# ibm-granite/dolomite-engine

Measured on AMD Instinct MI355X. Metric: tokens/sec/node GPTDolomite-3B bf16 seq4096 padding-free, higher is better.
Workload: dtype bf16; 1 GPU; gptdolomite-3b-bf16-seq4096-paddingfree-pretrain; model=GPTDolomite-3B, global_batch=16, seq_len=4096, parallelism=dp1

## Files before the change

### dolomite_engine_amd/csrc/attention.hip

```cpp

#include "common.h"

typedef __bf16 bf16x8 __attribute__((ext_vector_type(8)));
typedef float f32x4 __attribute__((ext_vector_type(4)));
typedef uint32_t u32x4 __attribute__((ext_vector_type(4)));

#define MFMA16(a, b, c) __builtin_amdgcn_mfma_f32_16x16x32_bf16((a), (b), (c), 0, 0, 0)

#define DOL_LOG2E 1.44269504088896340736f
#define DOL_LN2 0.69314718055994530942f

#define PI23(q) (((q) & ~12) | ((((q) >> 2) & 1) << 3) | ((((q) >> 3) & 1) << 2))

typedef __bf16 bf16x4 __attribute__((ext_vector_type(4)));


__device__ __forceinline__ bf16x8 lds_tr16_bfrag(const __bf16* img, int rowbase, int S, int d0, int lane) {
    const int g8 = (lane >> 4) * 8;
    const int jj = (lane >> 2) & 3;
    const int cc = (lane & 3) * 4;
    unsigned a0 = (unsigned)(size_t)(img + PI23(rowbase + g8 + jj) * S + d0 + cc);
    unsigned a1 = (unsigned)(size_t)(img + PI23(rowbase + g8 + 4 + jj) * S + d0 + cc);
    bf16x4 lo, hi;
    asm volatile(
// ... 381 lines not shown
    return dol_last_error();
}

static int fa_varlen_fwd_dispatch(dolomite_stream_t stream,
                                  const void* q, const void* k, const void* v,
                                  void* o, float* lse,
                                  const int32_t* seq_begin, const int32_t* seq_end,
                                  int batch, int max_seqlen, int64_t T,
                                  int H, int Hkv, int D, int G,
                                  int64_t q_tstride, int64_t q_gstride,
                                  int64_t k_tstride, int64_t k_hstride,
                                  int64_t v_tstride, int64_t v_hstride,
                                  float scale, int dtype, float p_drop, uint64_t seed) {
    if (dtype != DOLOMITE_BF16) return 9010;
    if (D > 128) return 9011;
    if (!(scale > 0.f)) return 9015;
    int max_tiles = (max_seqlen + 127) / 128;
    hipStream_t s = (hipStream_t)stream;
#define CASE(DP, DROP)                                                                               \
    return launch_fa_fwd<DP, DROP>(s, (const __bf16*)q, (const __bf16*)k, (const __bf16*)v,          \
                                   (__bf16*)o, lse, seq_begin, seq_end, batch, T, H, Hkv, D, G, q_tstride, \
                                   q_gstride, k_tstride, k_hstride, v_tstride, v_hstride, max_tiles, \
                                   scale, p_drop, seed)
    if (p_drop > 0.f) {
        if (D <= 32) CASE(32, true);
        if (D <= 64) CASE(64, true);
        if (D <= 96) CASE(96, true);
        CASE(128, true);
    }
    if (D <= 32) CASE(32, false);
    if (D <= 64) CASE(64, false);
    if (D <= 96) CASE(96, false);
    CASE(128, false);
#undef CASE
}

extern "C" int dolomite_fa_varlen_fwd(dolomite_stream_t stream,
                                      const void* q, const void* k, const void* v,
                                      void* o, float* lse,
                                      const int32_t* cu_seqlens, int batch, int max_seqlen, int64_t T,
                                      int H, int Hkv, int D, int G,
                                      int64_t q_tstride, int64_t q_gstride,
                                      int64_t k_tstride, int64_t k_hstride,
                                      int64_t v_tstride, int64_t v_hstride,
                                      float scale, int dtype) {
    return fa_varlen_fwd_dispatch(stream, q, k, v, o, lse, cu_seqlens, cu_seqlens + 1, batch, max_seqlen, T,
                                  H, Hkv, D, G, q_tstride, q_gstride, k_tstride, k_hstride,
                                  v_tstride, v_hstride, scale, dtype, 0.f, 0);
}

extern "C" int dolomite_fa_varlen_fwd_dropout(dolomite_stream_t stream,
                                              const void* q, const void* k, const void* v,
                                              void* o, float* lse,
                                              const int32_t* cu_seqlens, int batch, int max_seqlen, int64_t T,
                                              int H, int Hkv, int D, int G,
                                              int64_t q_tstride, int64_t q_gstride,
                                              int64_t k_tstride, int64_t k_hstride,
                                              int64_t v_tstride, int64_t v_hstride,
                                              float scale, int dtype, float p_drop, uint64_t seed) {
    if (!drop_p_valid(p_drop)) return 9013;
    return fa_varlen_fwd_dispatch(stream, q, k, v, o, lse, cu_seqlens, cu_seqlens + 1, batch, max_seqlen, T,
                                  H, Hkv, D, G, q_tstride, q_gstride, k_tstride, k_hstride,
                                  v_tstride, v_hstride, scale, dtype, p_drop, seed);
}


template <typename T>
__global__ void __launch_bounds__(256) fa_bwd_preprocess_kernel(
    const T* __restrict__ o, const T* __restrict__ dout, float* __restrict__ delta,
    int64_t T_total, int H, int D, int64_t o_ts, int64_t do_ts) {
    int64_t row = ((int64_t)blockIdx.x * 4) + (threadIdx.x >> 6);
    int lane = threadIdx.x & 63;
    if (row >= T_total * H) return;
    int64_t t = row / H;
    int h = (int)(row % H);
    const T* op = o + t * o_ts + (int64_t)h * D;
    const T* dp = dout + t * do_ts + (int64_t)h * D;
    float acc = 0.f;
    for (int d = lane * 2; d + 1 < D; d += 128) {
        float o0[2], d0[2];
        VecIO<T, 2>::load(op + d, o0);
        VecIO<T, 2>::load(dp + d, d0);
        acc += o0[0] * d0[0] + o0[1] * d0[1];
    }
    if (D & 1) {
        int d = D - 1;
        if (lane == 0) acc += load_as_f32(op + d) * load_as_f32(dp + d);
    }
    acc = wave_reduce_sum(acc);
    if (lane == 0) delta[(int64_t)h * T_total + t] = acc;
}

__global__ void __launch_bounds__(256) fa_bwd_preprocess_tiled(
    const __bf16* __restrict__ o, const __bf16* __restrict__ dout, float* __restrict__ delta,
    int64_t T_total, int H, int D, int TOK) {
    extern __shared__ float part[];
    const int64_t hd = (int64_t)H * D;
    const int64_t base = (int64_t)blockIdx.x * TOK * hd;
    const int64_t total = T_total * hd;
    const int np = (int)(TOK * hd / 8);
#pragma unroll 4
    for (int p = threadIdx.x; p < np; p += 256) {
        int64_t flat = base + (int64_t)p * 8;
        float acc = 0.f;
        if (flat + 8 <= total) {
            bf16x8 ov = *(const bf16x8*)(o + flat);
            bf16x8 dv = *(const bf16x8*)(dout + flat);
#pragma unroll
            for (int e = 0; e < 8; ++e) acc += (float)ov[e] * (float)dv[e];
        }
        part[p] = acc;
    }
    __syncthreads();
    const int slots = TOK * H;
    const int dp8 = D / 8;
    for (int s = threadIdx.x; s < slots; s += 256) {
        float a = 0.f;
        const float* ps = &part[s * dp8];
        for (int i = 0; i < dp8; ++i) a += ps[i];
        int tl = s / H, h = s - tl * H;
        int64_t t = (int64_t)blockIdx.x * TOK + tl;
        if (t < T_total) delta[(int64_t)h * T_total + t] = a;
    }
}

extern "C" int dolomite_fa_bwd_preprocess(dolomite_stream_t stream,
                                          const void* o, const void* dout, float* delta,
                                          int64_t T, int H, int D,
                                          int64_t o_tstride, int64_t do_tstride, int dtype) {
    const int64_t hd = (int64_t)H * D;
    int TOK = 16;
    while (TOK > 1 && TOK * hd * 4 / 8 > 65536) TOK /= 2;
    if (dtype == DOLOMITE_BF16 && D % 8 == 0 && o_tstride == hd && do_tstride == hd && T > 0 &&
        TOK * hd * 4 / 8 <= 65536) {
        dim3 grid((uint32_t)((T + TOK - 1) / TOK)), block(256);
        size_t shmem = (size_t)(TOK * hd / 8) * sizeof(float);
        hipLaunchKernelGGL((fa_bwd_preprocess_tiled), grid, block, shmem, (hipStream_t)stream,
                           (const __bf16*)o, (const __bf16*)dout, delta, T, H, D, TOK);
        return dol_last_error();
    }
    int64_t rows = T * H;
    dim3 grid((uint32_t)((rows + 3) / 4)), block(256);
    if (dtype == DOLOMITE_BF16)
        hipLaunchKernelGGL((fa_bwd_preprocess_kernel<uint16_t>), grid, block, 0, (hipStream_t)stream,
                           (const uint16_t*)o, (const uint16_t*)dout, delta, T, H, D, o_tstride, do_tstride);
    else
        hipLaunchKernelGGL((fa_bwd_preprocess_kernel<float>), grid, block, 0, (hipStream_t)stream,
                           (const float*)o, (const float*)dout, delta, T, H, D, o_tstride, do_tstride);
    return dol_last_error();
}



template <int DPAD, bool DROPOUT>
__global__ void __launch_bounds__(512, DPAD <= 96 ? 4 : 2) fa_bwd_dkv_kernel(
    const __bf16* __restrict__ q, const __bf16* __restrict__ k, const __bf16* __restrict__ v,
    const __bf16* __restrict__ dout, const float* __restrict__ lse, const float* __restrict__ delta,
    float* __restrict__ dk_acc, float* __restrict__ dv_acc,
    const int32_t* __restrict__ seq_begin, const int32_t* __restrict__ seq_end,
    int H, int Hkv, int D, int G,
    int64_t q_ts, int64_t q_gs, int64_t k_ts, int64_t k_hs, int64_t v_ts, int64_t v_hs,
    int64_t do_ts, int64_t T_total, float scale,
    uint32_t seed_lo, uint32_t seed_hi, uint32_t drop_thr, float drop_rp) {
    constexpr int KCH = DPAD / 32;
    constexpr int DCH = DPAD / 16;

    int tile_id = blockIdx.x, b = blockIdx.y, h = blockIdx.z;
    xcd_remap_tile_bh(tile_id, b, h);
    const int kvh = h / G;
    const int s0 = __builtin_amdgcn_readfirstlane(seq_begin[b]);
    const int L = __builtin_amdgcn_readfirstlane(seq_end[b]) - s0;
    const int ks = tile_id * 128;
    if (ks >= L) return;

    const int lane = threadIdx.x & 63;
    const int wave = threadIdx.x >> 6;
    const int lr = lane & 15;
    const int lg = lane >> 4;

    constexpr int SQ = DPAD + 16;
    constexpr int STS = 128 + 4;
    extern __shared__ char smem_raw[];
    __bf16* Qlds = (__bf16*)smem_raw;
    __bf16* dOl = Qlds + 64 * SQ;
    __bf16* dSTl = dOl + 64 * SQ;
    __bf16* PTl = dSTl + 64 * STS;

    const int kend = min(L, ks + 128);

    const int krow = ks + wave * 16 + lr;
    const bool kvalid = krow < kend;
    bf16x8 kfr[KCH], vfr[KCH];
#pragma unroll
    for (int kc = 0; kc < KCH; ++kc) {
        int d0 = kc * 32 + lg * 8;
        const __bf16* kp = k + (int64_t)(s0 + (kvalid ? krow : 0)) * k_ts + (int64_t)kvh * k_hs + d0;
        kfr[kc] = load_bf16x8_guard(kp, d0, D, kvalid);
        const __bf16* vp = v + (int64_t)(s0 + (kvalid ? krow : 0)) * v_ts + (int64_t)kvh * v_hs + d0;
        vfr[kc] = load_bf16x8_guard(vp, d0, D, kvalid);
    }

    f32x4 dvr[DCH], dkr[DCH];
#pragma unroll
    for (int dc = 0; dc < DCH; ++dc) {
        dvr[dc] = {0.f, 0.f, 0.f, 0.f};
        dkr[dc] = {0.f, 0.f, 0.f, 0.f};
    }

    uint32_t drop_cw[4];
    if constexpr (DROPOUT) {
        const uint32_t drop_hw = drop_head_word(seed_hi, (uint32_t)h);
#pragma unroll
        for (int r = 0; r < 4; ++r)
            drop_cw[r] = drop_col_word(drop_hw, (uint32_t)(s0 + ks + wave * 16 + lg * 4 + r));
    }

    const int tr_jj = (lane >> 2) & 3;
    const int tr_g8 = (lane >> 4) * 8;
    const int tr_cc = (lane & 3) * 4;
    const unsigned aQ0 = (unsigned)(size_t)(Qlds + PI23(tr_g8 + tr_jj) * SQ + tr_cc);
    const unsigned aQ1 = (unsigned)(size_t)(Qlds + PI23(tr_g8 + 4 + tr_jj) * SQ + tr_cc);
    const unsigned aDS0 = (unsigned)(size_t)(dSTl + PI23(tr_g8 + tr_jj) * STS + wave * 16 + tr_cc);
    const unsigned aDS1 = (unsigned)(size_t)(dSTl + PI23(tr_g8 + 4 + tr_jj) * STS + wave * 16 + tr_cc);
    constexpr int DO_IMM = 64 * SQ * 2;
    constexpr int PT_IMM = 64 * STS * 2;
    static_assert(DO_IMM + 32 * SQ * 2 + 16 * 2 < 65536, "ds offset range");
    static_assert(PT_IMM + 32 * STS * 2 + 16 * 2 < 65536, "ds offset range");

    if (__builtin_amdgcn_readfirstlane(threadIdx.x) >= 256) __builtin_amdgcn_s_setprio(1);

    const int qt0 = ks / 64;
    const int nqt = (L + 63) / 64;
    const int64_t q_hoff = (int64_t)(h / G) * q_gs + (int64_t)(h % G) * D;
    const int64_t do_hoff = (int64_t)h * D;

    if (D < DPAD) {
        for (int pidx = threadIdx.x; pidx < 64 * (DPAD - D) / 8; pidx += 512) {
            int qq = pidx / ((DPAD - D) / 8);
            int d0 = D + (pidx % ((DPAD - D) / 8)) * 8;
            bf16x8 z = {};
            *(bf16x8*)&Qlds[PI23(qq) * SQ + d0] = z;
            *(bf16x8*)&dOl[PI23(qq) * SQ + d0] = z;
        }
    }

    const unsigned st_magic = (1u << 22) / (unsigned)(D / 8) + 1;
    for (int qt = qt0; qt < nqt; ++qt) {
        const int qs = qt * 64;
        __syncthreads();
        {
            const int pieces = 64 * DPAD / 8;
            if (qs + 64 <= L) {
                for (int pidx = threadIdx.x; pidx < 64 * D / 8; pidx += 512) {
                    int qq = (int)(((unsigned)pidx * st_magic) >> 22);
                    int d0 = (pidx - qq * (D / 8)) * 8;
                    *(bf16x8*)&Qlds[PI23(qq) * SQ + d0] =
                        *(const bf16x8*)(q + (int64_t)(s0 + qs + qq) * q_ts + q_hoff + d0);
                    *(bf16x8*)&dOl[PI23(qq) * SQ + d0] =
                        *(const bf16x8*)(dout + (int64_t)(s0 + qs + qq) * do_ts + do_hoff + d0);
                }
            } else {
                for (int pidx = threadIdx.x; pidx < pieces; pidx += 512) {
                    int qq = pidx / (DPAD / 8);
                    int d0 = (pidx % (DPAD / 8)) * 8;
                    bool valid = (qs + qq) < L;
                    const __bf16* qp = q + (int64_t)(s0 + (valid ? qs + qq : 0)) * q_ts + q_hoff + d0;
                    *(bf16x8*)&Qlds[PI23(qq) * SQ + d0] = load_bf16x8_guard(qp, d0, D, valid);
                    const __bf16* dp = dout + (int64_t)(s0 + (valid ? qs + qq : 0)) * do_ts + do_hoff + d0;
                    *(bf16x8*)&dOl[PI23(qq) * SQ + d0] = load_bf16x8_guard(dp, d0, D, valid);
                }
            }
        }
        __syncthreads();

        const bool full_tile = (ks + wave * 16 + 16 <= qs + 1) && (kend == ks + 64) && (qs + 64 <= L);
#pragma unroll
        for (int cb = 0; cb < 4; ++cb) {
            f32x4 st = {0.f, 0.f, 0.f, 0.f};
            f32x4 dpt = {0.f, 0.f, 0.f, 0.f};
#pragma unroll
            for (int kc = 0; kc < KCH; ++kc) {
                int d0 = kc * 32 + lg * 8;
                bf16x8 qb = *(const bf16x8*)&Qlds[(cb * 16 + PI23(lr)) * SQ + d0];
                st = MFMA16(kfr[kc], qb, st);
                bf16x8 db = *(const bf16x8*)&dOl[(cb * 16 + PI23(lr)) * SQ + d0];
                dpt = MFMA16(vfr[kc], db, dpt);
            }
            const int qpos = qs + cb * 16 + lr;
            const bool qok = qpos < L;
            float lsev = qok ? lse[(int64_t)h * T_total + s0 + qpos] * DOL_LOG2E : 0.f;
            float delv = qok ? delta[(int64_t)h * T_total + s0 + qpos] : 0.f;
            bf16x4 pvv, dsv;
            uint32_t drop_rw = 0;
            if constexpr (DROPOUT) drop_rw = drop_row_word(seed_lo, (uint32_t)(s0 + qpos));
            if (__builtin_amdgcn_readfirstlane(full_tile ? 1 : 0)) {
#pragma unroll
                for (int r = 0; r < 4; ++r) {
                    float pv = exp2f(st[r] * (scale * DOL_LOG2E) - lsev);
                    if constexpr (DROPOUT) {
                        const bool keep = drop_keep_words(drop_rw, drop_cw[r], drop_thr);
                        pvv[r] = (__bf16)(keep ? pv : 0.f);
                        dsv[r] = (__bf16)(pv * ((keep ? dpt[r] * drop_rp : 0.f) - delv) * scale);
                    } else {
                        pvv[r] = (__bf16)pv;
                        dsv[r] = (__bf16)(pv * (dpt[r] - delv) * scale);
                    }
                }
            } else {
#pragma unroll
                for (int r = 0; r < 4; ++r) {
                    const int kpos = ks + wave * 16 + lg * 4 + r;
                    bool ok = qok && kpos < kend && kpos <= qpos;
                    float pv = ok ? exp2f(st[r] * (scale * DOL_LOG2E) - lsev) : 0.f;
                    if constexpr (DROPOUT) {
                        const bool keep = drop_keep_words(drop_rw, drop_cw[r], drop_thr);
                        float ds = ok ? pv * ((keep ? dpt[r] * drop_rp : 0.f) - delv) * scale : 0.f;
                        pvv[r] = (__bf16)(keep ? pv : 0.f);
                        dsv[r] = (__bf16)ds;
                    } else {
                        float ds = ok ? pv * (dpt[r] - delv) * scale : 0.f;
                        pvv[r] = (__bf16)pv;
                        dsv[r] = (__bf16)ds;
                    }
                }
            }
            const int srow = PI23(cb * 16 + lr) * STS + wave * 16 + lg * 4;
            *(bf16x4*)&PTl[srow] = pvv;
            *(bf16x4*)&dSTl[srow] = dsv;
        }

        {
            asm volatile("s_waitcnt lgkmcnt(0)" ::: "memory");
            __builtin_amdgcn_sched_barrier(0);
            bf16x4 a_lo[2], a_hi[2];
            tr16_issue<PT_IMM>(aDS0, aDS1, a_lo[0], a_hi[0]);
            tr16_issue<PT_IMM + 32 * STS * 2>(aDS0, aDS1, a_lo[1], a_hi[1]);
            bf16x4 blo[3], bhi[3];
            tr16_issue<DO_IMM>(aQ0, aQ1, blo[0], bhi[0]);
            tr16_issue<DO_IMM + ((1 / DCH) * 32 * SQ + (1 % DCH) * 16) * 2>(aQ0, aQ1, blo[1], bhi[1]);
            lgkm_wait4<4>(a_lo[0], a_hi[0], a_lo[1], a_hi[1]);
            bf16x8 af0 = tr16_join8(a_lo[0], a_hi[0]);
            bf16x8 af1 = tr16_join8(a_lo[1], a_hi[1]);
#define DKV_HALF(i, IMM, ACC, AF0, AF1)                                                                 \
    if constexpr ((i) < 2 * DCH) {                                                                      \
        constexpr int kc2_ = (i) / DCH, dc_ = (i) % DCH;                                                \
        if constexpr ((i) + 2 < 2 * DCH) {                                                              \
            constexpr int kn_ = ((i) + 2) / DCH, dn_ = ((i) + 2) % DCH;                                 \
            tr16_issue<(kn_ * 32 * SQ + dn_ * 16) * 2 + (IMM)>(aQ0, aQ1, blo[((i) + 2) % 3], bhi[((i) + 2) % 3]); \
            lgkm_wait2<4>(blo[(i) % 3], bhi[(i) % 3]);                                                  \
        } else if constexpr ((i) + 1 < 2 * DCH) {                                                       \
            lgkm_wait2<2>(blo[(i) % 3], bhi[(i) % 3]);                                                  \
        } else {                                                                                        \
            lgkm_wait2<0>(blo[(i) % 3], bhi[(i) % 3]);                                                  \
        }                                                                                               \
        ACC[dc_] = MFMA16(kc2_ ? (AF1) : (AF0), tr16_join8(blo[(i) % 3], bhi[(i) % 3]), ACC[dc_]);      \
    }
#define DKV_A(i) DKV_HALF(i, DO_IMM, dvr, af0, af1)
            DKV_A(0) DKV_A(1) DKV_A(2) DKV_A(3)
            DKV_A(4) DKV_A(5) DKV_A(6) DKV_A(7)
            DKV_A(8) DKV_A(9) DKV_A(10) DKV_A(11)
            DKV_A(12) DKV_A(13) DKV_A(14) DKV_A(15)
#undef DKV_A
            tr16_issue<0>(aDS0, aDS1, a_lo[0], a_hi[0]);
            tr16_issue<32 * STS * 2>(aDS0, aDS1, a_lo[1], a_hi[1]);
            tr16_issue<0>(aQ0, aQ1, blo[0], bhi[0]);
            tr16_issue<((1 / DCH) * 32 * SQ + (1 % DCH) * 16) * 2>(aQ0, aQ1, blo[1], bhi[1]);
            lgkm_wait4<4>(a_lo[0], a_hi[0], a_lo[1], a_hi[1]);
            af0 = tr16_join8(a_lo[0], a_hi[0]);
            af1 = tr16_join8(a_lo[1], a_hi[1]);
#define DKV_B(i) DKV_HALF(i, 0, dkr, af0, af1)
            DKV_B(0) DKV_B(1) DKV_B(2) DKV_B(3)
            DKV_B(4) DKV_B(5) DKV_B(6) DKV_B(7)
            DKV_B(8) DKV_B(9) DKV_B(10) DKV_B(11)
            DKV_B(12) DKV_B(13) DKV_B(14) DKV_B(15)
#undef DKV_B
#undef DKV_HALF
            __builtin_amdgcn_sched_barrier(0);
        }
    }

#pragma unroll
    for (int dc = 0; dc < DCH; ++dc) {
#pragma unroll
        for (int r = 0; r < 4; ++r) {
            const int kpos = ks + wave * 16 + lg * 4 + r;
            const int d = dc * 16 + lr;
            if (kpos < kend && d < D) {
                int64_t idx = ((int64_t)(s0 + kpos) * H + h) * D + d;
                __builtin_nontemporal_store(dkr[dc][r], &dk_acc[idx]);
                if constexpr (DROPOUT)
                    __builtin_nontemporal_store(dvr[dc][r] * drop_rp, &dv_acc[idx]);
                else
                    __builtin_nontemporal_store(dvr[dc][r], &dv_acc[idx]);
            }
        }
    }
}

template <int DPAD, bool DROPOUT>
__global__ void __launch_bounds__(512, (DROPOUT && DPAD > 96) ? 2 : 4) fa_bwd_dq_kernel(
    const __bf16* __restrict__ q, const __bf16* __restrict__ k, const __bf16* __restrict__ v,
    const __bf16* __restrict__ dout, const float* __restrict__ lse, const float* __restrict__ delta,
    __bf16* __restrict__ dqkv_q,
    const int32_t* __restrict__ seq_begin, const int32_t* __restrict__ seq_end,
    int H, int Hkv, int D, int G,
    int64_t q_ts, int64_t q_gs, int64_t k_ts, int64_t k_hs, int64_t v_ts, int64_t v_hs,
    int64_t do_ts, int64_t T_total, float scale,
    uint32_t seed_lo, uint32_t seed_hi, uint32_t drop_thr, float drop_rp) {
    constexpr int KCH = DPAD / 32;
    constexpr int DCH = DPAD / 16;

    int tile_id = blockIdx.x, b = blockIdx.y, h = blockIdx.z;
    xcd_remap_tile_bh(tile_id, b, h);
    const int kvh = h / G;
    const int s0 = __builtin_amdgcn_readfirstlane(seq_begin[b]);
    const int L = __builtin_amdgcn_readfirstlane(seq_end[b]) - s0;
    const int ntile_seq = (L + 127) / 128;
    if (tile_id >= ntile_seq) return;
    const int qs = (ntile_seq - 1 - tile_id) * 128;

    const int lane = threadIdx.x & 63;
    const int wave = threadIdx.x >> 6;
    const int lr = lane & 15;
    const int lg = lane >> 4;

    constexpr int SQ = FaKvLds<DPAD>::S;
    extern __shared__ char smem_raw[];
    __bf16* Klds = (__bf16*)smem_raw;
    __bf16* Vlds = Klds + 64 * SQ;
    uint32_t* Cw = (uint32_t*)(Vlds + 64 * SQ);

    const int64_t q_hoff = (int64_t)(h / G) * q_gs + (int64_t)(h % G) * D;
    const int64_t do_hoff = (int64_t)h * D;

    unsigned aK0, aK1;
    fa_tr16_perm_bases(Klds, SQ, lane, aK0, aK1);

    const int qrow = qs + wave * 16 + lr;
    const bool qvalid = qrow < L;
    bf16x8 qfr[KCH], dfr[KCH];
#pragma unroll
    for (int kc = 0; kc < KCH; ++kc) {
        int d0 = kc * 32 + lg * 8;
        const __bf16* qp = q + (int64_t)(s0 + (qvalid ? qrow : 0)) * q_ts + q_hoff + d0;
        qfr[kc] = load_bf16x8_guard(qp, d0, D, qvalid);
        const __bf16* dp = dout + (int64_t)(s0 + (qvalid ? qrow : 0)) * do_ts + do_hoff + d0;
        dfr[kc] = load_bf16x8_guard(dp, d0, D, qvalid);
    }

    const float lsev = qvalid ? lse[(int64_t)h * T_total + s0 + qrow] * DOL_LOG2E : 0.f;
    const float delv = qvalid ? delta[(int64_t)h * T_total + s0 + qrow] : 0.f;
    const float scale2 = scale * DOL_LOG2E;

    f32x4 dq[DCH];
#pragma unroll
    for (int dc = 0; dc < DCH; ++dc) dq[dc] = {0.f, 0.f, 0.f, 0.f};

    uint32_t drop_rw = 0;
    uint32_t drop_hw = 0;
    if constexpr (DROPOUT) {
        drop_hw = drop_head_word(seed_hi, (uint32_t)h);
        drop_rw = drop_row_word(seed_lo, (uint32_t)(s0 + qrow));
    }

    if (D < DPAD) {
        for (int pidx = threadIdx.x; pidx < 64 * (DPAD - D) / 8; pidx += 512) {
            int key = pidx / ((DPAD - D) / 8);
            int d0 = D + (pidx % ((DPAD - D) / 8)) * 8;
            bf16x8 z = {};
            *(bf16x8*)&Klds[key * SQ + d0] = z;
            *(bf16x8*)&Vlds[key * SQ + d0] = z;
        }
    }

    int st_koff[2], st_voff[2];
    int st_klds[2], st_vlds[2];
#pragma unroll
    for (int j = 0; j < 2; ++j) {
        int pidx = (int)threadIdx.x + j * 512;
        int pp = pidx < 64 * D / 8 ? pidx : 0;
        int key = pp / (D / 8);
        int d0 = (pp % (D / 8)) * 8;
        st_koff[j] = (int)(key * k_ts + kvh * k_hs) + d0;
        st_voff[j] = (int)(key * v_ts + kvh * v_hs) + d0;
        st_klds[j] = key * SQ + d0;
        st_vlds[j] = key * SQ + d0;
    }

    const int kend_total = min(L, qs + 128);
    const int nkt = (kend_total + 63) / 64;

    if (__builtin_amdgcn_readfirstlane(threadIdx.x) >= 256) __builtin_amdgcn_s_setprio(1);

    for (int kt = 0; kt < nkt; ++kt) {
        const int ks = kt * 64;
        __syncthreads();
        {
            const int pieces = 64 * DPAD / 8;
            if (ks + 64 <= kend_total) {
                const int64_t disp = (int64_t)(s0 + ks);
#pragma unroll
                for (int j = 0; j < 2; ++j) {
                    if ((int)threadIdx.x + j * 512 < 64 * D / 8) {
                        *(bf16x8*)&Klds[st_klds[j]] = *(const bf16x8*)(k + disp * k_ts + st_koff[j]);
                        *(bf16x8*)&Vlds[st_vlds[j]] = *(const bf16x8*)(v + disp * v_ts + st_voff[j]);
                    }
                }
            } else {
                for (int pidx = threadIdx.x; pidx < pieces; pidx += 512) {
                    int key = pidx / (DPAD / 8);
                    int d0 = (pidx % (DPAD / 8)) * 8;
                    bool valid = (ks + key) < kend_total;
                    const __bf16* kp = k + (int64_t)(s0 + (valid ? ks + key : 0)) * k_ts + (int64_t)kvh * k_hs + d0;
                    *(bf16x8*)&Klds[key * SQ + d0] = load_bf16x8_guard(kp, d0, D, valid);
                    const __bf16* vp = v + (int64_t)(s0 + (valid ? ks + key : 0)) * v_ts + (int64_t)kvh * v_hs + d0;
                    *(bf16x8*)&Vlds[key * SQ + d0] = load_bf16x8_guard(vp, d0, D, valid);
                }
            }
            if constexpr (DROPOUT) {
                if (__builtin_amdgcn_readfirstlane(threadIdx.x) < 64)
                    Cw[lane] = drop_col_word(drop_hw, (uint32_t)(s0 + ks + lane));
            }
        }
        __syncthreads();

        const bool full_tile = (ks + 64 <= qs + wave * 16 + 1) && (ks + 64 <= kend_total) && (qs + wave * 16 + 16 <= L);
        bf16x8 dsf[2];
#pragma unroll
        for (int cb = 0; cb < 4; ++cb) {
            f32x4 sc = {0.f, 0.f, 0.f, 0.f};
            f32x4 dp = {0.f, 0.f, 0.f, 0.f};
#pragma unroll
            for (int kc = 0; kc < KCH; ++kc) {
                int d0 = kc * 32 + lg * 8;
                bf16x8 kb = *(const bf16x8*)&Klds[(cb * 16 + lr) * SQ + d0];
                sc = MFMA16(kb, qfr[kc], sc);
                bf16x8 vb = *(const bf16x8*)&Vlds[(cb * 16 + lr) * SQ + d0];
                dp = MFMA16(vb, dfr[kc], dp);
            }
            u32x4 cw = {};
            if constexpr (DROPOUT) cw = *(const u32x4*)&Cw[cb * 16 + lg * 4];
            if (__builtin_amdgcn_readfirstlane(full_tile ? 1 : 0)) {
#pragma unroll
                for (int x = 0; x < 4; ++x) {
                    float pv = exp2f(fmaf(sc[x], scale2, -lsev));
                    float dpm = dp[x];
                    if constexpr (DROPOUT)
                        dpm = drop_keep_words(drop_rw, cw[x], drop_thr) ? dp[x] * drop_rp : 0.f;
                    dsf[cb >> 1][(cb & 1) * 4 + x] = (__bf16)(pv * (dpm - delv) * scale);
                }
            } else {
#pragma unroll
                for (int x = 0; x < 4; ++x) {
                    const int kpos = ks + cb * 16 + lg * 4 + x;
                    bool ok = qvalid && kpos < kend_total && kpos <= qrow;
                    float pv = ok ? exp2f(fmaf(sc[x], scale2, -lsev)) : 0.f;
                    float dpm = dp[x];
                    if constexpr (DROPOUT)
                        dpm = drop_keep_words(drop_rw, cw[x], drop_thr) ? dp[x] * drop_rp : 0.f;
                    float ds = ok ? pv * (dpm - delv) * scale : 0.f;
                    dsf[cb >> 1][(cb & 1) * 4 + x] = (__bf16)ds;
                }
            }
        }

        {
            __builtin_amdgcn_sched_barrier(0);
            bf16x4 klo[4], khi[4];
            tr16_issue<0>(aK0, aK1, klo[0], khi[0]);
            tr16_issue<((1 / DCH) * 32 * SQ + (1 % DCH) * 16) * 2>(aK0, aK1, klo[1], khi[1]);
            tr16_issue<((2 / DCH) * 32 * SQ + (2 % DCH) * 16) * 2>(aK0, aK1, klo[2], khi[2]);
#define DQ_STEP(i)                                                                                      \
    if constexpr ((i) < 2 * DCH) {                                                                      \
        constexpr int kc2_ = (i) / DCH, dc_ = (i) % DCH;                                                \
        if constexpr ((i) + 3 < 2 * DCH) {                                                              \
            constexpr int kn_ = ((i) + 3) / DCH, dn_ = ((i) + 3) % DCH;                                 \
            tr16_issue<(kn_ * 32 * SQ + dn_ * 16) * 2>(aK0, aK1, klo[((i) + 3) % 4], khi[((i) + 3) % 4]); \
            lgkm_wait2<6>(klo[(i) % 4], khi[(i) % 4]);                                                  \
        } else if constexpr ((i) + 2 < 2 * DCH) {                                                       \
            lgkm_wait2<4>(klo[(i) % 4], khi[(i) % 4]);                                                  \
        } else if constexpr ((i) + 1 < 2 * DCH) {                                                       \
            lgkm_wait2<2>(klo[(i) % 4], khi[(i) % 4]);                                                  \
        } else {                                                                                        \
            lgkm_wait2<0>(klo[(i) % 4], khi[(i) % 4]);                                                  \
        }                                                                                               \
        dq[dc_] = MFMA16(tr16_join8(klo[(i) % 4], khi[(i) % 4]), dsf[kc2_], dq[dc_]);                   \
    }
            DQ_STEP(0) DQ_STEP(1) DQ_STEP(2) DQ_STEP(3)
            DQ_STEP(4) DQ_STEP(5) DQ_STEP(6) DQ_STEP(7)
            DQ_STEP(8) DQ_STEP(9) DQ_STEP(10) DQ_STEP(11)
            DQ_STEP(12) DQ_STEP(13) DQ_STEP(14) DQ_STEP(15)
#undef DQ_STEP
            __builtin_amdgcn_sched_barrier(0);
        }
    }

    __bf16* dqrow = dqkv_q + (int64_t)(s0 + (qvalid ? qrow : 0)) * q_ts + q_hoff;
#pragma unroll
    for (int dc = 0; dc < DCH; ++dc) {
        const int d0 = dc * 16 + lg * 4;
        bf16x4 dv;
#pragma unroll
        for (int x = 0; x < 4; ++x) dv[x] = (__bf16)dq[dc][x];
        if (qvalid && d0 < D) *(bf16x4*)&dqrow[d0] = dv;
    }
}

template <int DPAD, bool DROPOUT>
static int launch_fa_bwd(hipStream_t stream, const __bf16* q, const __bf16* k, const __bf16* v,
                         const __bf16* dout, const float* lse, const float* delta,
                         __bf16* dqkv_q, float* dk_acc, float* dv_acc,
                         const int32_t* seq_begin, const int32_t* seq_end,
                         int batch, int64_t T, int H, int Hkv, int D, int G,
                         int64_t q_ts, int64_t q_gs, int64_t k_ts, int64_t k_hs,
                         int64_t v_ts, int64_t v_hs, int64_t do_ts, int max_tiles, float scale,
                         float p_drop, uint64_t seed) {
    dim3 block(512);
    dim3 grid(max_tiles, batch, H);
    constexpr int SQ = DPAD + 16;
    const uint32_t seed_lo = (uint32_t)seed, seed_hi = (uint32_t)(seed >> 32);
    const uint32_t thr = drop_threshold(p_drop);
    const float rp = 1.f / (1.f - p_drop);
    size_t shmem_dkv = (size_t)(64 * (128 + 4) * 2 + 64 * SQ * 2) * sizeof(__bf16);
    hipLaunchKernelGGL((fa_bwd_dkv_kernel<DPAD, DROPOUT>), grid, block, shmem_dkv, stream,
                       q, k, v, dout, lse, delta, dk_acc, dv_acc, seq_begin, seq_end, H, Hkv, D, G,
                       q_ts, q_gs, k_ts, k_hs, v_ts, v_hs, do_ts, T, scale,
                       seed_lo, seed_hi, thr, rp);
    int err = dol_last_error();
    if (err) return err;
    hipLaunchKernelGGL((fa_bwd_dq_kernel<DPAD, DROPOUT>), grid, block, FaKvLds<DPAD>::bytes(DROPOUT), stream,
                       q, k, v, dout, lse, delta, dqkv_q, seq_begin, seq_end, H, Hkv, D, G,
                       q_ts, q_gs, k_ts, k_hs, v_ts, v_hs, do_ts, T, scale,
                       seed_lo, seed_hi, thr, rp);
    return dol_last_error();
}

static int fa_varlen_bwd_dispatch(dolomite_stream_t stream,
                                  const void* q, const void* k, const void* v,
                                  const void* dout, const float* lse,
                                  const float* delta, void* dqkv_q, float* dk_acc, float* dv_acc,
                                  const int32_t* seq_begin, const int32_t* seq_end,
                                  int batch, int max_seqlen, int64_t T,
                                  int H, int Hkv, int D, int G,
                                  int64_t q_tstride, int64_t q_gstride,
                                  int64_t k_tstride, int64_t k_hstride,
                                  int64_t v_tstride, int64_t v_hstride,
                                  int64_t do_tstride,
                                  float scale, int dtype, float p_drop, uint64_t seed) {
    if (dtype != DOLOMITE_BF16) return 9010;
    if (D > 128) return 9011;
    int max_tiles = (max_seqlen + 127) / 128;
    hipStream_t s = (hipStream_t)stream;
#define CASE(DP, DROP)                                                                                  \
    return launch_fa_bwd<DP, DROP>(s, (const __bf16*)q, (const __bf16*)k, (const __bf16*)v,             \
                                   (const __bf16*)dout, lse, delta, (__bf16*)dqkv_q, dk_acc, dv_acc,    \
                                   seq_begin, seq_end, batch, T, H, Hkv, D, G, q_tstride, q_gstride, k_tstride, \
                                   k_hstride, v_tstride, v_hstride, do_tstride, max_tiles, scale,       \
                                   p_drop, seed)
    if (p_drop > 0.f) {
        if (D <= 32) CASE(32, true);
        if (D <= 64) CASE(64, true);
        if (D <= 96) CASE(96, true);
        CASE(128, true);
    }
    if (D <= 32) CASE(32, false);
    if (D <= 64) CASE(64, false);
    if (D <= 96) CASE(96, false);
    CASE(128, false);
#undef CASE
}

extern "C" int dolomite_fa_varlen_bwd(dolomite_stream_t stream,
                                      const void* q, const void* k, const void* v,
                                      const void* dout, const float* lse,
                                      const float* delta, void* dqkv_q, float* dk_acc, float* dv_acc,
                                      const int32_t* cu_seqlens, int batch, int max_seqlen, int64_t T,
                                      int H, int Hkv, int D, int G,
                                      int64_t q_tstride, int64_t q_gstride,
                                      int64_t k_tstride, int64_t k_hstride,
                                      int64_t v_tstride, int64_t v_hstride,
                                      int64_t do_tstride,
                                      float scale, int dtype) {
    return fa_varlen_bwd_dispatch(stream, q, k, v, dout, lse, delta, dqkv_q, dk_acc, dv_acc,
                                  cu_seqlens, cu_seqlens + 1, batch, max_seqlen, T, H, Hkv, D, G,
                                  q_tstride, q_gstride, k_tstride, k_hstride, v_tstride, v_hstride,
                                  do_tstride, scale, dtype, 0.f, 0);
}

extern "C" int dolomite_fa_varlen_bwd_dropout(dolomite_stream_t stream,
                                              const void* q, const void* k, const void* v,
                                              const void* dout, const float* lse,
                                              const float* delta, void* dqkv_q, float* dk_acc, float* dv_acc,
                                              const int32_t* cu_seqlens, int batch, int max_seqlen, int64_t T,
                                              int H, int Hkv, int D, int G,
                                              int64_t q_tstride, int64_t q_gstride,
                                              int64_t k_tstride, int64_t k_hstride,
                                              int64_t v_tstride, int64_t v_hstride,
                                              int64_t do_tstride,
                                              float scale, int dtype, float p_drop, uint64_t seed) {
    if (!drop_p_valid(p_drop)) return 9013;
    return fa_varlen_bwd_dispatch(stream, q, k, v, dout, lse, delta, dqkv_q, dk_acc, dv_acc,
                                  cu_seqlens, cu_seqlens + 1, batch, max_seqlen, T, H, Hkv, D, G,
                                  q_tstride, q_gstride, k_tstride, k_hstride, v_tstride, v_hstride,
                                  do_tstride, scale, dtype, p_drop, seed);
}


__global__ void __launch_bounds__(256) fa_zero_gap_rows_kernel(
    uint4* __restrict__ buf, int64_t row_vec,
    const int32_t* __restrict__ seq_begin, const int32_t* __restrict__ seq_end,
    int batch, int64_t T) {
    const int g = blockIdx.y;
    int64_t lo = g == 0 ? 0 : (int64_t)seq_end[g - 1];
    int64_t hi = g == batch ? T : (int64_t)seq_begin[g];
    lo = lo < 0 ? 0 : lo;
    hi = hi > T ? T : hi;
    if (hi <= lo) return;
    const int64_t first = lo * row_vec, last = hi * row_vec;
    const uint4 z = {0u, 0u, 0u, 0u};
    for (int64_t i = first + (int64_t)blockIdx.x * 256 + threadIdx.x; i < last;
         i += (int64_t)gridDim.x * 256)
        buf[i] = z;
}

extern "C" int dolomite_fa_zero_gap_rows(dolomite_stream_t stream, void* buf, int64_t row_bytes,
                                         const int32_t* seq_begin, const int32_t* seq_end,
                                         int batch, int64_t T) {
    if (row_bytes <= 0 || row_bytes % 16 != 0) return 9016;
    if (batch < 0 || T < 0 || batch >= 65535) return 9014;
    if (T == 0) return 0;
    const int64_t vec_per_gap = (T * (row_bytes / 16) + batch) / (batch + 1);
    int64_t chunks = (vec_per_gap + 1023) / 1024;
    chunks = chunks < 1 ? 1 : (chunks > 1024 ? 1024 : chunks);
    hipLaunchKernelGGL(fa_zero_gap_rows_kernel, dim3((uint32_t)chunks, (uint32_t)(batch + 1)),
                       dim3(256), 0, (hipStream_t)stream, (uint4*)buf, row_bytes / 16,
                       seq_begin, seq_end, batch, T);
    return dol_last_error();
}

extern "C" int dolomite_fa_spans_fwd(dolomite_stream_t stream,
                                     const void* q, const void* k, const void* v,
                                     void* o, float* lse,
                                     const int32_t* seq_begin, const int32_t* seq_end,
                                     int batch, int max_seqlen, int64_t T,
                                     int H, int Hkv, int D, int G,
                                     int64_t q_tstride, int64_t q_gstride,
                                     int64_t k_tstride, int64_t k_hstride,
                                     int64_t v_tstride, int64_t v_hstride,
                                     float scale, int dtype, float p_drop, uint64_t seed) {
    if (!drop_p_valid(p_drop)) return 9013;
    if (dtype != DOLOMITE_BF16) return 9010;
    if (D > 128) return 9011;
    if (!(scale > 0.f)) return 9015;
    int err = dolomite_fa_zero_gap_rows(stream, o, (int64_t)H * D * (int64_t)sizeof(__bf16),
                                        seq_begin, seq_end, batch, T);
    if (err) return err;
    if (batch == 0 || max_seqlen <= 0) return 0;
    return fa_varlen_fwd_dispatch(stream, q, k, v, o, lse, seq_begin, seq_end, batch, max_seqlen, T,
                                  H, Hkv, D, G, q_tstride, q_gstride, k_tstride, k_hstride,
                                  v_tstride, v_hstride, scale, dtype, p_drop, seed);
}

extern "C" int dolomite_fa_spans_bwd(dolomite_stream_t stream,
                                     const void* q, const void* k, const void* v,
                                     const void* dout, const float* lse,
                                     const float* delta, void* dqkv_q, float* dk_acc, float* dv_acc,
                                     const int32_t* seq_begin, const int32_t* seq_end,
                                     int batch, int max_seqlen, int64_t T,
                                     int H, int Hkv, int D, int G,
                                     int64_t q_tstride, int64_t q_gstride,
                                     int64_t k_tstride, int64_t k_hstride,
                                     int64_t v_tstride, int64_t v_hstride,
                                     int64_t do_tstride,
                                     float scale, int dtype, float p_drop, uint64_t seed) {
    if (!drop_p_valid(p_drop)) return 9013;
    if (dtype != DOLOMITE_BF16) return 9010;
    if (D > 128) return 9011;
// ... 157 lines not shown
```

Measured before the change: 50110 tokens/s.

## Keep P and dS in registers in flash-attention dK/dV backward kernel

```diff
diff --git a/dolomite_engine_amd/csrc/attention.hip b/dolomite_engine_amd/csrc/attention.hip
--- a/dolomite_engine_amd/csrc/attention.hip
+++ b/dolomite_engine_amd/csrc/attention.hip
@@ -557,6 +557,18 @@
 
 
 
+
+__device__ __forceinline__ float dkv_exp2(float x) { return __builtin_amdgcn_exp2f(x); }
+
+template <int DPAD>
+struct FaDkvLds {
+    static constexpr int S = DPAD + 16;
+    static constexpr size_t image_bytes = (size_t)2 * 64 * S * sizeof(__bf16);
+    static constexpr size_t bytes(bool dropout) {
+        return image_bytes + 2 * 64 * sizeof(float) + (dropout ? 64 * sizeof(uint32_t) : 0);
+    }
+};
+
 template <int DPAD, bool DROPOUT>
 __global__ void __launch_bounds__(512, DPAD <= 96 ? 4 : 2) fa_bwd_dkv_kernel(
     const __bf16* __restrict__ q, const __bf16* __restrict__ k, const __bf16* __restrict__ v,
@@ -583,13 +595,13 @@
     const int lr = lane & 15;
     const int lg = lane >> 4;
 
-    constexpr int SQ = DPAD + 16;
-    constexpr int STS = 128 + 4;
+    constexpr int SQ = FaDkvLds<DPAD>::S;
     extern __shared__ char smem_raw[];
     __bf16* Qlds = (__bf16*)smem_raw;
     __bf16* dOl = Qlds + 64 * SQ;
-    __bf16* dSTl = dOl + 64 * SQ;
-    __bf16* PTl = dSTl + 64 * STS;
+    float* Lsel = (float*)(dOl + 64 * SQ);
+    float* NDel = Lsel + 64;
+    uint32_t* Rw = (uint32_t*)(NDel + 64);
 
     const int kend = min(L, ks + 128);
 
@@ -612,25 +624,15 @@
         dkr[dc] = {0.f, 0.f, 0.f, 0.f};
     }
 
-    uint32_t drop_cw[4];
-    if constexpr (DROPOUT) {
-        const uint32_t drop_hw = drop_head_word(seed_hi, (uint32_t)h);
-#pragma unroll
-        for (int r = 0; r < 4; ++r)
-            drop_cw[r] = drop_col_word(drop_hw, (uint32_t)(s0 + ks + wave * 16 + lg * 4 + r));
-    }
-
-    const int tr_jj = (lane >> 2) & 3;
-    const int tr_g8 = (lane >> 4) * 8;
-    const int tr_cc = (lane & 3) * 4;
-    const unsigned aQ0 = (unsigned)(size_t)(Qlds + PI23(tr_g8 + tr_jj) * SQ + tr_cc);
-    const unsigned aQ1 = (unsigned)(size_t)(Qlds + PI23(tr_g8 + 4 + tr_jj) * SQ + tr_cc);
-    const unsigned aDS0 = (unsigned)(size_t)(dSTl + PI23(tr_g8 + tr_jj) * STS + wave * 16 + tr_cc);
-    const unsigned aDS1 = (unsigned)(size_t)(dSTl + PI23(tr_g8 + 4 + tr_jj) * STS + wave * 16 + tr_cc);
+    uint32_t drop_cw = 0;
+    if constexpr (DROPOUT)
+        drop_cw = drop_col_word(drop_head_word(seed_hi, (uint32_t)h), (uint32_t)(s0 + krow));
+
+    unsigned aQ0, aQ1;
+    fa_tr16_perm_bases(Qlds, SQ, lane, aQ0, aQ1);
     constexpr int DO_IMM = 64 * SQ * 2;
-    constexpr int PT_IMM = 64 * STS * 2;
-    static_assert(DO_IMM + 32 * SQ * 2 + 16 * 2 < 65536, "ds offset range");
-    static_assert(PT_IMM + 32 * STS * 2 + 16 * 2 < 65536, "ds offset range");
+    static_assert(DO_IMM + 32 * SQ * 2 + DPAD * 2 < 65536, "ds offset range");
+    const float scale2 = scale * DOL_LOG2E;
 
     if (__builtin_amdgcn_readfirstlane(threadIdx.x) >= 256) __builtin_amdgcn_s_setprio(1);
 
@@ -644,10 +646,98 @@
             int qq = pidx / ((DPAD - D) / 8);
             int d0 = D + (pidx % ((DPAD - D) / 8)) * 8;
             bf16x8 z = {};
-            *(bf16x8*)&Qlds[PI23(qq) * SQ + d0] = z;
-            *(bf16x8*)&dOl[PI23(qq) * SQ + d0] = z;
-        }
-    }
+            *(bf16x8*)&Qlds[qq * SQ + d0] = z;
+            *(bf16x8*)&dOl[qq * SQ + d0] = z;
+        }
+    }
+
+    auto dkv_chunk = [&](auto cc, const int qs, const int full) {
+        constexpr int c = decltype(cc)::value;
+        bf16x8 pf, dsf;
+#pragma unroll
+        for (int hb = 0; hb < 2; ++hb) {
+            const int cb = 2 * c + hb;
+            f32x4 st = {0.f, 0.f, 0.f, 0.f};
+            f32x4 dpt = {0.f, 0.f, 0.f, 0.f};
+            if constexpr (!DROPOUT) dpt = *(const f32x4*)&NDel[cb * 16 + lg * 4];
+#pragma unroll
+            for (int kc = 0; kc < KCH; ++kc) {
+                int d0 = kc * 32 + lg * 8;
+                bf16x8 qa = *(const bf16x8*)&Qlds[(cb * 16 + lr) * SQ + d0];
+                st = MFMA16(qa, kfr[kc], st);
+                bf16x8 da = *(const bf16x8*)&dOl[(cb * 16 + lr) * SQ + d0];
+                dpt = MFMA16(da, vfr[kc], dpt);
+            }
+            const f32x4 ls = *(const f32x4*)&Lsel[cb * 16 + lg * 4];
+            u32x4 rw = {};
+            f32x4 nd = {};
+            if constexpr (DROPOUT) {
+                rw = *(const u32x4*)&Rw[cb * 16 + lg * 4];
+                nd = *(const f32x4*)&NDel[cb * 16 + lg * 4];
+            }
+            if (full) {
+#pragma unroll
+                for (int x = 0; x < 4; ++x) {
+                    float pv = dkv_exp2(fmaf(st[x], scale2, -ls[x]));
+                    if constexpr (DROPOUT) {
+                        const bool keep = drop_keep_words(rw[x], drop_cw, drop_thr);
+                        pf[hb * 4 + x] = (__bf16)(keep ? pv : 0.f);
+                        dsf[hb * 4 + x] = (__bf16)(pv * fmaf(keep ? dpt[x] : 0.f, drop_rp, nd[x]));
+                    } else {
+                        pf[hb * 4 + x] = (__bf16)pv;
+                        dsf[hb * 4 + x] = (__bf16)(pv * dpt[x]);
+                    }
+                }
+            } else {
+#pragma unroll
+                for (int x = 0; x < 4; ++x) {
+                    const int qpos = qs + cb * 16 + lg * 4 + x;
+                    const bool ok = kvalid && qpos < L && krow <= qpos;
+                    float pv = ok ? dkv_exp2(fmaf(st[x], scale2, -ls[x])) : 0.f;
+                    if constexpr (DROPOUT) {
+                        const bool keep = drop_keep_words(rw[x], drop_cw, drop_thr);
+                        float ds = ok ? pv * fmaf(keep ? dpt[x] : 0.f, drop_rp, nd[x]) : 0.f;
+                        pf[hb * 4 + x] = (__bf16)(keep ? pv : 0.f);
+                        dsf[hb * 4 + x] = (__bf16)ds;
+                    } else {
+                        float ds = ok ? pv * dpt[x] : 0.f;
+                        pf[hb * 4 + x] = (__bf16)pv;
+                        dsf[hb * 4 + x] = (__bf16)ds;
+                    }
+                }
+            }
+        }
+
+        __builtin_amdgcn_sched_barrier(0);
+        constexpr int CB = c * 32 * SQ * 2;
+        bf16x4 alo[3], ahi[3];
+        tr16_issue<CB + DO_IMM>(aQ0, aQ1, alo[0], ahi[0]);
+        static_assert(DCH >= 2, "fragment 1 is the dO image's second 16-col block");
+        tr16_issue<CB + DO_IMM + 32>(aQ0, aQ1, alo[1], ahi[1]);
+#define DKV_STEP(i)                                                                                     \
+    if constexpr ((i) < 2 * DCH) {                                                                      \
+        constexpr int im_ = (i) / DCH, dc_ = (i) % DCH;                                                 \
+        if constexpr ((i) + 2 < 2 * DCH) {                                                              \
+            constexpr int in_ = ((i) + 2) / DCH, dn_ = ((i) + 2) % DCH;                                 \
+            tr16_issue<CB + (in_ ? 0 : DO_IMM) + dn_ * 32>(aQ0, aQ1, alo[((i) + 2) % 3], ahi[((i) + 2) % 3]); \
+            lgkm_wait2<4>(alo[(i) % 3], ahi[(i) % 3]);                                                  \
+        } else if constexpr ((i) + 1 < 2 * DCH) {                                                       \
+            lgkm_wait2<2>(alo[(i) % 3], ahi[(i) % 3]);                                                  \
+        } else {                                                                                        \
+            lgkm_wait2<0>(alo[(i) % 3], ahi[(i) % 3]);                                                  \
+        }                                                                                               \
+        if constexpr (im_ == 0)                                                                         \
+            dvr[dc_] = MFMA16(tr16_join8(alo[(i) % 3], ahi[(i) % 3]), pf, dvr[dc_]);                    \
+        else                                                                                            \
+            dkr[dc_] = MFMA16(tr16_join8(alo[(i) % 3], ahi[(i) % 3]), dsf, dkr[dc_]);                   \
+    }
+        DKV_STEP(0) DKV_STEP(1) DKV_STEP(2) DKV_STEP(3)
+        DKV_STEP(4) DKV_STEP(5) DKV_STEP(6) DKV_STEP(7)
+        DKV_STEP(8) DKV_STEP(9) DKV_STEP(10) DKV_STEP(11)
+        DKV_STEP(12) DKV_STEP(13) DKV_STEP(14) DKV_STEP(15)
+#undef DKV_STEP
+        __builtin_amdgcn_sched_barrier(0);
+    };
 
     const unsigned st_magic = (1u << 22) / (unsigned)(D / 8) + 1;
     for (int qt = qt0; qt < nqt; ++qt) {
@@ -659,9 +749,9 @@
                 for (int pidx = threadIdx.x; pidx < 64 * D / 8; pidx += 512) {
                     int qq = (int)(((unsigned)pidx * st_magic) >> 22);
                     int d0 = (pidx - qq * (D / 8)) * 8;
-                    *(bf16x8*)&Qlds[PI23(qq) * SQ + d0] =
+                    *(bf16x8*)&Qlds[qq * SQ + d0] =
                         *(const bf16x8*)(q + (int64_t)(s0 + qs + qq) * q_ts + q_hoff + d0);
-                    *(bf16x8*)&dOl[PI23(qq) * SQ + d0] =
+                    *(bf16x8*)&dOl[qq * SQ + d0] =
                         *(const bf16x8*)(dout + (int64_t)(s0 + qs + qq) * do_ts + do_hoff + d0);
                 }
             } else {
@@ -670,134 +760,40 @@
                     int d0 = (pidx % (DPAD / 8)) * 8;
                     bool valid = (qs + qq) < L;
                     const __bf16* qp = q + (int64_t)(s0 + (valid ? qs + qq : 0)) * q_ts + q_hoff + d0;
-                    *(bf16x8*)&Qlds[PI23(qq) * SQ + d0] = load_bf16x8_guard(qp, d0, D, valid);
+                    *(bf16x8*)&Qlds[qq * SQ + d0] = load_bf16x8_guard(qp, d0, D, valid);
                     const __bf16* dp = dout + (int64_t)(s0 + (valid ? qs + qq : 0)) * do_ts + do_hoff + d0;
-                    *(bf16x8*)&dOl[PI23(qq) * SQ + d0] = load_bf16x8_guard(dp, d0, D, valid);
+                    *(bf16x8*)&dOl[qq * SQ + d0] = load_bf16x8_guard(dp, d0, D, valid);
                 }
             }
+            const int swave = __builtin_amdgcn_readfirstlane(wave);
+            const bool sok = qs + lane < L;
+            const int64_t sidx = (int64_t)h * T_total + s0 + (sok ? qs + lane : 0);
+            if (swave == 0) {
+                Lsel[lane] = sok ? lse[sidx] * DOL_LOG2E : 0.f;
+            } else if (swave == 1) {
+                NDel[lane] = sok ? -delta[sidx] : 0.f;
+            } else if (swave == 2) {
+                if constexpr (DROPOUT) Rw[lane] = drop_row_word(seed_lo, (uint32_t)(s0 + qs + lane));
+            }
         }
         __syncthreads();
 
-        const bool full_tile = (ks + wave * 16 + 16 <= qs + 1) && (kend == ks + 64) && (qs + 64 <= L);
-#pragma unroll
-        for (int cb = 0; cb < 4; ++cb) {
-            f32x4 st = {0.f, 0.f, 0.f, 0.f};
-            f32x4 dpt = {0.f, 0.f, 0.f, 0.f};
-#pragma unroll
-            for (int kc = 0; kc < KCH; ++kc) {
-                int d0 = kc * 32 + lg * 8;
-                bf16x8 qb = *(const bf16x8*)&Qlds[(cb * 16 + PI23(lr)) * SQ + d0];
-                st = MFMA16(kfr[kc], qb, st);
-                bf16x8 db = *(const bf16x8*)&dOl[(cb * 16 + PI23(lr)) * SQ + d0];
-                dpt = MFMA16(vfr[kc], db, dpt);
-            }
-            const int qpos = qs + cb * 16 + lr;
-            const bool qok = qpos < L;
-            float lsev = qok ? lse[(int64_t)h * T_total + s0 + qpos] * DOL_LOG2E : 0.f;
-            float delv = qok ? delta[(int64_t)h * T_total + s0 + qpos] : 0.f;
-            bf16x4 pvv, dsv;
-            uint32_t drop_rw = 0;
-            if constexpr (DROPOUT) drop_rw = drop_row_word(seed_lo, (uint32_t)(s0 + qpos));
-            if (__builtin_amdgcn_readfirstlane(full_tile ? 1 : 0)) {
-#pragma unroll
-                for (int r = 0; r < 4; ++r) {
-                    float pv = exp2f(st[r] * (scale * DOL_LOG2E) - lsev);
-                    if constexpr (DROPOUT) {
-                        const bool keep = drop_keep_words(drop_rw, drop_cw[r], drop_thr);
-                        pvv[r] = (__bf16)(keep ? pv : 0.f);
-                        dsv[r] = (__bf16)(pv * ((keep ? dpt[r] * drop_rp : 0.f) - delv) * scale);
-                    } else {
-                        pvv[r] = (__bf16)pv;
-                        dsv[r] = (__bf16)(pv * (dpt[r] - delv) * scale);
-                    }
-                }
-            } else {
-#pragma unroll
-                for (int r = 0; r < 4; ++r) {
-                    const int kpos = ks + wave * 16 + lg * 4 + r;
-                    bool ok = qok && kpos < kend && kpos <= qpos;
-                    float pv = ok ? exp2f(st[r] * (scale * DOL_LOG2E) - lsev) : 0.f;
-                    if constexpr (DROPOUT) {
-                        const bool keep = drop_keep_words(drop_rw, drop_cw[r], drop_thr);
-                        float ds = ok ? pv * ((keep ? dpt[r] * drop_rp : 0.f) - delv) * scale : 0.f;
-                        pvv[r] = (__bf16)(keep ? pv : 0.f);
-                        dsv[r] = (__bf16)ds;
-                    } else {
-                        float ds = ok ? pv * (dpt[r] - delv) * scale : 0.f;
-                        pvv[r] = (__bf16)pv;
-                        dsv[r] = (__bf16)ds;
-                    }
-                }
-            }
-            const int srow = PI23(cb * 16 + lr) * STS + wave * 16 + lg * 4;
-            *(bf16x4*)&PTl[srow] = pvv;
-            *(bf16x4*)&dSTl[srow] = dsv;
-        }
-
-        {
-            asm volatile("s_waitcnt lgkmcnt(0)" ::: "memory");
-            __builtin_amdgcn_sched_barrier(0);
-            bf16x4 a_lo[2], a_hi[2];
-            tr16_issue<PT_IMM>(aDS0, aDS1, a_lo[0], a_hi[0]);
-            tr16_issue<PT_IMM + 32 * STS * 2>(aDS0, aDS1, a_lo[1], a_hi[1]);
-            bf16x4 blo[3], bhi[3];
-            tr16_issue<DO_IMM>(aQ0, aQ1, blo[0], bhi[0]);
-            tr16_issue<DO_IMM + ((1 / DCH) * 32 * SQ + (1 % DCH) * 16) * 2>(aQ0, aQ1, blo[1], bhi[1]);
-            lgkm_wait4<4>(a_lo[0], a_hi[0], a_lo[1], a_hi[1]);
-            bf16x8 af0 = tr16_join8(a_lo[0], a_hi[0]);
-            bf16x8 af1 = tr16_join8(a_lo[1], a_hi[1]);
-#define DKV_HALF(i, IMM, ACC, AF0, AF1)                                                                 \
-    if constexpr ((i) < 2 * DCH) {                                                                      \
-        constexpr int kc2_ = (i) / DCH, dc_ = (i) % DCH;                                                \
-        if constexpr ((i) + 2 < 2 * DCH) {                                                              \
-            constexpr int kn_ = ((i) + 2) / DCH, dn_ = ((i) + 2) % DCH;                                 \
-            tr16_issue<(kn_ * 32 * SQ + dn_ * 16) * 2 + (IMM)>(aQ0, aQ1, blo[((i) + 2) % 3], bhi[((i) + 2) % 3]); \
-            lgkm_wait2<4>(blo[(i) % 3], bhi[(i) % 3]);                                                  \
-        } else if constexpr ((i) + 1 < 2 * DCH) {                                                       \
-            lgkm_wait2<2>(blo[(i) % 3], bhi[(i) % 3]);                                                  \
-        } else {                                                                                        \
-            lgkm_wait2<0>(blo[(i) % 3], bhi[(i) % 3]);                                                  \
-        }                                                                                               \
-        ACC[dc_] = MFMA16(kc2_ ? (AF1) : (AF0), tr16_join8(blo[(i) % 3], bhi[(i) % 3]), ACC[dc_]);      \
-    }
-#define DKV_A(i) DKV_HALF(i, DO_IMM, dvr, af0, af1)
-            DKV_A(0) DKV_A(1) DKV_A(2) DKV_A(3)
-            DKV_A(4) DKV_A(5) DKV_A(6) DKV_A(7)
-            DKV_A(8) DKV_A(9) DKV_A(10) DKV_A(11)
-            DKV_A(12) DKV_A(13) DKV_A(14) DKV_A(15)
-#undef DKV_A
-            tr16_issue<0>(aDS0, aDS1, a_lo[0], a_hi[0]);
-            tr16_issue<32 * STS * 2>(aDS0, aDS1, a_lo[1], a_hi[1]);
-            tr16_issue<0>(aQ0, aQ1, blo[0], bhi[0]);
-            tr16_issue<((1 / DCH) * 32 * SQ + (1 % DCH) * 16) * 2>(aQ0, aQ1, blo[1], bhi[1]);
-            lgkm_wait4<4>(a_lo[0], a_hi[0], a_lo[1], a_hi[1]);
-            af0 = tr16_join8(a_lo[0], a_hi[0]);
-            af1 = tr16_join8(a_lo[1], a_hi[1]);
-#define DKV_B(i) DKV_HALF(i, 0, dkr, af0, af1)
-            DKV_B(0) DKV_B(1) DKV_B(2) DKV_B(3)
-            DKV_B(4) DKV_B(5) DKV_B(6) DKV_B(7)
-            DKV_B(8) DKV_B(9) DKV_B(10) DKV_B(11)
-            DKV_B(12) DKV_B(13) DKV_B(14) DKV_B(15)
-#undef DKV_B
-#undef DKV_HALF
-            __builtin_amdgcn_sched_barrier(0);
-        }
-    }
-
+        const bool full_tile = (ks + wave * 16 + 16 <= qs + 1) && (ks + wave * 16 + 16 <= kend) && (qs + 64 <= L);
+        const int full = __builtin_amdgcn_readfirstlane(full_tile ? 1 : 0);
+        dkv_chunk(std::integral_constant<int, 0>{}, qs, full);
+        dkv_chunk(std::integral_constant<int, 1>{}, qs, full);
+    }
+
+    const int64_t rowoff = ((int64_t)(s0 + (kvalid ? krow : 0)) * H + h) * D;
 #pragma unroll
     for (int dc = 0; dc < DCH; ++dc) {
-#pragma unroll
-        for (int r = 0; r < 4; ++r) {
-            const int kpos = ks + wave * 16 + lg * 4 + r;
-            const int d = dc * 16 + lr;
-            if (kpos < kend && d < D) {
-                int64_t idx = ((int64_t)(s0 + kpos) * H + h) * D + d;
-                __builtin_nontemporal_store(dkr[dc][r], &dk_acc[idx]);
-                if constexpr (DROPOUT)
-                    __builtin_nontemporal_store(dvr[dc][r] * drop_rp, &dv_acc[idx]);
-                else
-                    __builtin_nontemporal_store(dvr[dc][r], &dv_acc[idx]);
-            }
+        const int d0 = dc * 16 + lg * 4;
+        if (kvalid && d0 < D) {
+            f32x4 dkv4 = dkr[dc] * scale;
+            __builtin_nontemporal_store(dkv4, (f32x4*)&dk_acc[rowoff + d0]);
+            f32x4 dvv4 = dvr[dc];
+            if constexpr (DROPOUT) dvv4 *= drop_rp;
+            __builtin_nontemporal_store(dvv4, (f32x4*)&dv_acc[rowoff + d0]);
         }
     }
 }
@@ -1022,12 +1018,10 @@
                          float p_drop, uint64_t seed) {
     dim3 block(512);
     dim3 grid(max_tiles, batch, H);
-    constexpr int SQ = DPAD + 16;
     const uint32_t seed_lo = (uint32_t)seed, seed_hi = (uint32_t)(seed >> 32);
     const uint32_t thr = drop_threshold(p_drop);
     const float rp = 1.f / (1.f - p_drop);
-    size_t shmem_dkv = (size_t)(64 * (128 + 4) * 2 + 64 * SQ * 2) * sizeof(__bf16);
-    hipLaunchKernelGGL((fa_bwd_dkv_kernel<DPAD, DROPOUT>), grid, block, shmem_dkv, stream,
+    hipLaunchKernelGGL((fa_bwd_dkv_kernel<DPAD, DROPOUT>), grid, block, FaDkvLds<DPAD>::bytes(DROPOUT), stream,
                        q, k, v, dout, lse, delta, dk_acc, dv_acc, seq_begin, seq_end, H, Hkv, D, G,
                        q_ts, q_gs, k_ts, k_hs, v_ts, v_hs, do_ts, T, scale,
                        seed_lo, seed_hi, thr, rp);
```

New measurement: 51950 tokens/s (median of 6 runs). +3.7%, better.
